# anton-galkovsky/pointcloudTraj

Measured on AMD Instinct MI355X. Metric: nn_queries_per_sec_10M_point_cloud, higher is better.
Workload: dtype f64; 1 GPU; C3-throughput: 10000000 uniform fp32 points in [0,100.0)^3 (seed 3), 1048576 uniform NN queries per step (4 distinct batches in rotation, seeds [5, 1005, 2005, 3005]), grid kernel, inputs resident in HBM; points_per_gpu=10000000, total_points=10000000, algo=grid, query_batches_in_rotation=4, gpu_work_before_the_warmup_steps=none, full=False, parallelism=single GPU, cards=1

## Files before the change

pointcloudtraj_amd/build.py:

```python
from __future__ import annotations

import os
import shutil
import subprocess

PKG = os.path.dirname(os.path.abspath(__file__))
ROOT = os.path.dirname(PKG)
CSRC = os.path.join(PKG, "csrc")
LIB = os.path.join(PKG, "lib")
ENGINE_SO = os.environ.get("PCT_ENGINE_SO") or os.path.join(LIB, "libpct_engine.so")
KDTREE_SO = os.path.join(LIB, "libkdtree.so")
DEMO_BIN = os.path.join(LIB, "seam_demo")
NODE_BIN = os.path.join(LIB, "node_call_sites")
CORRIDOR_SO = os.path.join(LIB, "libpct_corridor.so")
SHARD_SO = os.path.join(LIB, "libpct_shard.so")
SHARD_CLIENT = os.path.join(LIB, "shard_client")

HIPCC = shutil.which("hipcc") or "/opt/rocm/bin/hipcc"
COMMON = ["-O3", "--offload-arch=gfx950", "-std=c++17", "-fPIC", "-shared", "-ffp-contract=off",
          "-Wall", "-Wno-unused-function", "-I" + os.path.join(ROOT, "include")]


def _stale(target: str, sources: list[str]) -> bool:
    if not os.path.exists(target):
        return True
    t = os.path.getmtime(target)
    return any(os.path.getmtime(s) > t for s in sources)


def build_all(force: bool = False, verbose: bool = False) -> None:
    os.makedirs(LIB, exist_ok=True)
    hdrs = [os.path.join(ROOT, "include", "pct_engine.h"), os.path.join(ROOT, "include", "kdtree", "kdtree.h"),
            os.path.join(ROOT, "include", "kdtree", "kdtree_ext.h")]
    hdrs += [os.path.join(ROOT, "include", "pct_voxel.h"), os.path.join(ROOT, "include", "pct_traj.h")]
    eng_units = [os.path.join(CSRC, "engine.hip"), os.path.join(CSRC, "voxel.hip"), os.path.join(CSRC, "traj.hip"), os.path.join(CSRC, "nodeset.hip")]
    eng_src = eng_units + [os.path.join(CSRC, f) for f in ("kernels.hpp", "gridbuild.hpp", "pyramid.hpp", "bernstein.hpp", "brute2.hpp", "knn.hpp", "rsearch.hpp", "ring.hpp", "ring_dedup.hpp", "vox_key.hpp", "ring_search.hpp", "ring_host.inc", "engine_internal.hpp")]
    if force or _stale(ENGINE_SO, eng_src + hdrs):
        cmd = [HIPCC, *COMMON, "-o", ENGINE_SO, *eng_units]
        if verbose:
            print(" ".join(cmd))
        subprocess.run(cmd, check=True)
    kd_src = [os.path.join(CSRC, "kdtree_gpu.cpp")]
    if os.path.exists(kd_src[0]) and (force or _stale(KDTREE_SO, kd_src + hdrs + [ENGINE_SO])):
        cmd = ["g++", "-O2", "-std=c++17", "-fPIC", "-shared", "-Wall", "-ffp-contract=off", "-I" + os.path.join(ROOT, "include"),
               "-o", KDTREE_SO, kd_src[0], "-L" + LIB, "-lpct_engine", "-Wl,-rpath,$ORIGIN", "-Wl,-soname,libkdtree.so"]
        if verbose:
            print(" ".join(cmd))
        subprocess.run(cmd, check=True)


    cor_src = os.path.join(CSRC, "corridor.cpp")
    cor_hdrs = [os.path.join(ROOT, "include", h) for h in ("pct_corridor.h", "pct_corridor_finder.hpp", "pct_obstacle_map.hpp")]
    if os.path.exists(cor_src) and os.path.exists(KDTREE_SO) and (force or _stale(CORRIDOR_SO, [cor_src, KDTREE_SO] + cor_hdrs + hdrs)):
        cmd = ["g++", "-O2", "-std=c++17", "-fPIC", "-shared", "-Wall", "-ffp-contract=off", "-I" + os.path.join(ROOT, "include"),
               "-o", CORRIDOR_SO, cor_src, "-L" + LIB, "-lkdtree", "-lpct_engine", "-Wl,-rpath,$ORIGIN", "-Wl,-rpath-link," + LIB,
               "-L/opt/rocm/lib", "-Wl,-rpath-link,/opt/rocm/lib", "-Wl,-soname,libpct_corridor.so"]
        if verbose:
            print(" ".join(cmd))
        subprocess.run(cmd, check=True)
# ... 57 lines not shown
```

pointcloudtraj_amd/csrc/engine.hip:

```cpp
#include <hip/hip_runtime.h>
#include <hip/hip_ext.h>

#include <algorithm>
#include <chrono>
#include <cmath>
#include <cstdarg>
#include <cstdio>
#include <cstdlib>
#include <cstring>
#include <type_traits>
#include <vector>

#include "../../include/pct_engine.h"
#include "engine_internal.hpp"
#include "kernels.hpp"
#include "gridbuild.hpp"
#include "pyramid.hpp"
#include "ring.hpp"
#include "ring_dedup.hpp"
#include "brute2.hpp"
#include "knn.hpp"
#include "rsearch.hpp"
#include "ring_search.hpp"

// ... 126 lines not shown
    ExpandOut *h_eout = nullptr, *d_eout = nullptr;
    double *h_bpos = nullptr, *d_bpos = nullptr;
    unsigned char *d_stage = nullptr;
    size_t stage_bytes = 0;
    float *d_bbox = nullptr;
    GbCheck *d_gbcheck = nullptr, *h_gbcheck = nullptr;
    GbCheck last_check{};
    bool has_pyr = false;
    PyrDesc P{};
    PyrNode *pyr_nodes = nullptr;
    unsigned char *pyr_hint = nullptr;
    size_t pyr_cap = 0, pyr_total = 0, pyr_hint_cap = 0;
    double empty_frac = 0.0;
    bool was_sparse = false;
    bool has_grid = false;
    GridDesc G{};
    uint32_t *cell_start = nullptr;
    size_t cells_cap = 0;
    float4 *sorted = nullptr;
    size_t sorted_cap = 0;
    uint4 *blocks = nullptr;
    size_t blocks_cap = 0;
    BinDesc B{};
    float4 *d_qsorted = nullptr;
    uint32_t *d_sort1 = nullptr;
    int sort_phase = 0;
    int64_t qcap = 0;
    float *d_q = nullptr, *d_r = nullptr;
    double *d_q64 = nullptr, *d_r2 = nullptr, *d_d2 = nullptr, *d_radius = nullptr, *d_pts64 = nullptr;
    uint32_t *d_idx = nullptr, *d_count = nullptr, *d_bound = nullptr;
    uint32_t *d_todo = nullptr;
    unsigned char *d_skip = nullptr;
    double *d_part_d2 = nullptr;
    uint32_t *d_part_idx = nullptr;
    int64_t part_q = 0;
    uint32_t *d_ovf = nullptr;
    uint32_t *d_cand_count = nullptr, *d_cand_idx = nullptr;
    double *d_cand_d2 = nullptr;
    uint32_t *d_knn_idx = nullptr, *d_knn_pidx = nullptr;
    double *d_knn_d2 = nullptr, *d_knn_pd2 = nullptr;
    size_t knn_out_cap = 0, knn_part_cap = 0;
    long long *rs_off = nullptr;
    uint64_t *rs_tiles = nullptr;
    uint32_t *rs_cursor = nullptr, *rs_queue = nullptr;
    int64_t rs_qcap = 0;
    uint32_t *rs_idx = nullptr;
// ... 519 lines not shown
    const double *d_q64 = c->d_q64 + 3 * qoff;
    d_idx += qoff;
    d_d2 += qoff;
    const int blocks = stream_blocks(c->count, Q);
    return launch_frame(c, s, Q, { Work::EveryPoint }, no_step,
        [&] {
            for_each_query_tile(Q, [&](auto qt, int q0, int qcount) {
                nn_stream_kernel<decltype(qt)::value><<<blocks, 256, 0, s>>>(c->x, c->y, c->z, (uint32_t)c->count, d_q64, q0, qcount, c->d_part_d2,
                                                                             c->d_part_idx, blocks);
            });
        },
        [&] {
            nn_reduce_partials_kernel<<<(int)Q, 256, 0, s>>>(c->d_part_d2, c->d_part_idx, blocks, (uint32_t)c->index_base, d_idx, d_d2);
        });
}

int nn_stream_q64(pct_cloud *c, int64_t Q, uint32_t *d_idx, double *d_d2, hipStream_t s)
{
    for (int64_t off = 0; off < Q; off += c->part_q) PCTCHK(nn_stream_q64_slice(c, off, std::min<int64_t>(c->part_q, Q - off), d_idx, d_d2, s));
    c->host_points = (uint64_t)Q * (uint64_t)c->count;
    return PCT_OK;
}

int bin_queries(pct_cloud *c, const float *d_q, int64_t Q, hipStream_t s, const float4 **recs_out)
{
    *recs_out = nullptr;
    if (Q < 16384) return PCT_OK;
    const BinDesc &B = c->B;
    int key_shift = 0;
    while ((((uint64_t)B.nbins - 1) >> key_shift) >= (1ull << 20)) key_shift++;
    const bool pingpong = !c->capturing;
    uint32_t *total1 = c->d_sort1 + (c->sort_phase ? kSortBuckets : 0), *total1_next = c->d_sort1 + (c->sort_phase ? 0 : kSortBuckets);
    uint32_t *fill1 = c->d_sort1 + 2 * kSortBuckets;
    const uint32_t per_block = (uint32_t)std::min<int64_t>(kSortPerBlock, std::max<int64_t>(1024, (Q / 128 + 1023) / 1024 * 1024));
    const int nb = ceil_div(Q, (int64_t)per_block);
    with_bool((reinterpret_cast<uintptr_t>(d_q) & 15u) == 0, [&](auto aligned) {
        constexpr bool A = decltype(aligned)::value;
        qsort_hist_kernel<A><<<nb, 1024, 0, s>>>(c->G, B, key_shift, d_q, (uint32_t)Q, per_block, total1, fill1, pingpong ? total1_next : nullptr);
        qsort_scatter1_kernel<A><<<nb, 1024, 0, s>>>(c->G, B, key_shift, d_q, (uint32_t)Q, per_block, total1, fill1, c->d_qsorted);
    });
    if (pingpong) c->sort_phase ^= 1;
    else HIPCHK(hipMemsetAsync(total1, 0, sizeof(uint32_t) * kSortBuckets, s));
    HIPCHK(hipGetLastError());
    *recs_out = c->d_qsorted;
    return PCT_OK;
}

int g_filter_mode = -1;

int cloud_bbox_cached(pct_cloud *c)
{
    if (c->bbox_epoch == c->content_epoch) return PCT_OK;
    hipStream_t s = g_stream;
    const int64_t n = c->count;
    const int bblocks = (int)std::min<int64_t>(1024, (n + 255) / 256);
    float *d_part = c->d_bbox;
    bbox_partial_kernel<<<bblocks, 256, 0, s>>>(c->x, c->y, c->z, (uint32_t)n, d_part);
    std::vector<float> part((size_t)bblocks * 6);
    hipError_t e = hipMemcpyAsync(part.data(), d_part, part.size() * sizeof(float), hipMemcpyDeviceToHost, s);
    if (e == hipSuccess) e = hipStreamSynchronize(s);
    if (e != hipSuccess) return fail(PCT_ERR_HIP, "bbox reduction failed: %s", hipGetErrorString(e));
    for (int k = 0; k < 3; k++) { c->bbox_lo[k] = INFINITY; c->bbox_hi[k] = -INFINITY; }
// ... 147 lines not shown
        return fail(PCT_ERR_INVALID, "unknown algo %d", algo);
    }
    if (op == Op::KNN && *path == Path::Stream && c->capturing)
        return fail(PCT_ERR_INVALID, "the streaming k-NN kernel is not available during graph capture");
    if (c->count == 0) *path = Path::Empty;
    return PCT_OK;
}

int nn_run(pct_cloud *c, Path path, const float *d_q, int64_t Q, uint32_t *d_idx, double *d_d2, hipStream_t s)
{
    switch (path) {
    case Path::Empty:
        fill_empty_kernel<<<ceil_div(Q, 256), 256, 0, s>>>(d_idx, d_d2, (uint32_t)Q);
        HIPCHK(hipGetLastError());
        return PCT_OK;
    case Path::Table:
        return launch_frame(c, s, Q, { Work::DeviceKept }, [&] {
            ring_batch_kernel<false><<<(int)Q, 256, 0, s>>>(ring_view(c), InflateParams{}, d_q, nullptr, (double)INFINITY, (uint32_t)c->index_base, d_idx, d_d2,
                                                            nullptr, nullptr, ExpressSignal{});
        });
    case Path::Grid: {
        const float4 *recs = nullptr;
        const int blocks = ceil_div(Q, 256 / kCoop);
        return launch_frame(c, s, Q, { Work::Device, Dom::Ext }, [&] { return bin_queries(c, d_q, Q, s, &recs); },
            [&] {
                with_bool(c->count_work, [&](auto count_work) {
                    constexpr bool CW = decltype(count_work)::value;
                    if (c->has_pyr) {
                        launch_dominant(c, s, nn_grid_pyr_kernel<CW>, blocks, c->G, c->P, c->pyr_nodes, c->pyr_hint, c->sorted, c->cell_start, d_q, (uint32_t)Q,
                                        (uint32_t)c->index_base, recs, d_idx, d_d2, c->d_work, c->d_todo);
                        nn_grid_pyr_todo_kernel<CW><<<(int)std::min<int64_t>(256, blocks), 256, 0, s>>>(c->G, c->P, c->pyr_nodes, c->pyr_hint, c->sorted, c->cell_start, d_q,
                                                                                                        (uint32_t)c->index_base, recs, d_idx, d_d2, c->d_work, c->d_todo);
                    } else
                        launch_dominant(c, s, nn_grid_coop_kernel<CW>, blocks, c->G, c->sorted, c->cell_start, d_q, (uint32_t)Q, (uint32_t)c->index_base, recs, d_idx,
                                        d_d2, c->d_work);
                });
            }, no_step);
    }
    default:
        widen_queries_kernel<<<ceil_div(3 * Q, 256), 256, 0, s>>>(d_q, (uint32_t)(3 * Q), c->d_q64);
        if (path == Path::StreamExact) return nn_stream_q64(c, Q, d_idx, d_d2, s);
        return nn_stream_filtered(c, d_q, Q, d_idx, d_d2, s);
    }
}

int nn_dev(pct_cloud *c, int algo, const float *d_q, int64_t Q, uint32_t *d_idx, double *d_d2, hipStream_t s)
{
    if (Q == 0) return PCT_OK;
    if (Q > c->qcap) return fail(PCT_ERR_INVALID, "batch of %lld exceeds reserved %lld (call pct_cloud_reserve_queries)", (long long)Q, (long long)c->qcap);
    Path path;
    PCTCHK(resolve_algo(c, Op::NN, algo, Q, &path));
    return nn_run(c, path, d_q, Q, d_idx, d_d2, s);
}

int count_run(pct_cloud *c, Path path, const float *d_q, const float *d_r, int64_t Q, uint32_t *d_count, hipStream_t s)
{
    HIPCHK(hipMemsetAsync(d_count, 0, sizeof(uint32_t) * Q, s));
    switch (path) {
// ... 372 lines not shown
        if (c->hx) (void)hipHostFree(c->hx);
        if (c->hy) (void)hipHostFree(c->hy);
        if (c->hz) (void)hipHostFree(c->hz);
        c->x = c->y = c->z = nullptr;
    }
    if (c->h_xout) (void)hipHostFree(c->h_xout);
    if (c->h_xin) (void)hipHostFree(c->h_xin);
    if (c->h_xr) (void)hipHostFree(c->h_xr);
    if (c->h_xids) (void)hipHostFree(c->h_xids);
    if (c->h_xseq) (void)hipHostFree(c->h_xseq);
    if (c->ev_mut) (void)hipEventDestroy(c->ev_mut);
    if (c->h_frame) (void)hipHostFree(c->h_frame);
    if (c->h_astage) (void)hipHostFree(c->h_astage);
    if (c->h_mq) (void)hipHostFree(c->h_mq);
    if (c->h_mi) (void)hipHostFree(c->h_mi);
    if (c->h_md) (void)hipHostFree(c->h_md);
    dev_free(c->d_xcounter);
    if (c->h_aux) (void)hipHostFree(c->h_aux);
    if (c->h_eout) (void)hipHostFree(c->h_eout);
    if (c->h_bpos) (void)hipHostFree(c->h_bpos);
    dev_free(c->x); dev_free(c->y); dev_free(c->z); dev_free(c->d_stage); dev_free(c->gb_tmp); dev_free(c->gb_small);
    dev_free(c->blocks);
    dev_free(c->cell_start); dev_free(c->sorted);
    dev_free(c->d_qsorted); dev_free(c->d_sort1); dev_free(c->d_todo);
    dev_free(c->d_q); dev_free(c->d_r); dev_free(c->d_q64); dev_free(c->d_r2); dev_free(c->d_d2); dev_free(c->d_radius);
    dev_free(c->d_pts64); dev_free(c->d_idx); dev_free(c->d_count); dev_free(c->d_skip); dev_free(c->d_bound);
    dev_free(c->d_part_d2); dev_free(c->d_part_idx); dev_free(c->d_cand_count); dev_free(c->d_cand_d2); dev_free(c->d_cand_idx); dev_free(c->d_ovf);
    dev_free(c->d_coef); dev_free(c->d_segtime); dev_free(c->d_orders); dev_free(c->d_nsamples); dev_free(c->d_first_hit);
    dev_free(c->d_work);
    dev_free(c->d_knn_idx); dev_free(c->d_knn_d2); dev_free(c->d_knn_pidx); dev_free(c->d_knn_pd2);
    dev_free(c->rs_off); dev_free(c->rs_tiles); dev_free(c->rs_cursor); dev_free(c->rs_queue); dev_free(c->rs_idx); dev_free(c->rs_d2);
    dev_free(c->d_bbox); dev_free(c->d_gbcheck); dev_free(c->pyr_nodes); dev_free(c->pyr_hint);
    if (c->h_gbcheck) (void)hipHostFree(c->h_gbcheck);
    dev_free(c->ring_ht); dev_free(c->ring_slots); dev_free(c->ring_ovf); dev_free(c->ring_where); dev_free(c->ring_st);
    if (c->h_ring_status) (void)hipHostFree(c->h_ring_status);
    dev_free(c->dd_keys); dev_free(c->dd_vals); dev_free(c->dd_pslot); dev_free(c->dd_rank); dev_free(c->dd_tile); dev_free(c->dd_flags); dev_free(c->dd_out);
    if (c->h_dd_word) (void)hipHostFree(c->h_dd_word);
    replan_ctx_free(c->rp);
    dev_free(c->crop_tile); dev_free(c->crop_idx); dev_free(c->crop_d2); dev_free(c->crop_x); dev_free(c->crop_y); dev_free(c->crop_z);
    if (c->ev0) (void)hipEventDestroy(c->ev0);
    if (c->ev1) (void)hipEventDestroy(c->ev1);
    for (hipEvent_t e : c->dom_ring) if (e) (void)hipEventDestroy(e);
    delete c;
    return PCT_OK;
}

int64_t pct_cloud_size(const pct_cloud *c) { return c ? c->count : 0; }
// ... 73 lines not shown

extern "C" {

int pct_cloud_append_aos(pct_cloud *c, const void *pts, int64_t n, int64_t stride_bytes)
{
    if (!c || n < 0 || (n > 0 && !pts) || stride_bytes < 12 || (stride_bytes & 3)) return fail(PCT_ERR_INVALID, "bad append arguments");
    if (n > c->cap) return fail(PCT_ERR_CAPACITY, "appending %lld points to a ring of %lld", (long long)n, (long long)c->cap);
    if (c->ring_on && c->dd_res > 0) return ring_append_dedup(c, pts, n, stride_bytes);
    if (n == 0) return PCT_OK;
    drop_grid(c);
    if (c->ring_ready) return ring_append(c, pts, n, stride_bytes);
    return append_unindexed(c, pts, n, stride_bytes);
}

int pct_cloud_reserve_queries(pct_cloud *c, int64_t Q)
{
    if (!c || Q < 0) return fail(PCT_ERR_INVALID, "bad reserve");
    if (Q <= c->qcap) return PCT_OK;
    if (c->capturing) return fail(PCT_ERR_INVALID, "cannot grow workspaces during graph capture");
    HIPCHK(hipStreamSynchronize(g_stream));
    const int64_t q = std::max<int64_t>(Q, 256);
    dev_free(c->d_q); dev_free(c->d_r); dev_free(c->d_q64); dev_free(c->d_r2); dev_free(c->d_d2); dev_free(c->d_radius);
    dev_free(c->d_pts64); dev_free(c->d_idx); dev_free(c->d_count); dev_free(c->d_skip); dev_free(c->d_bound);
    dev_free(c->d_part_d2); dev_free(c->d_part_idx); dev_free(c->d_cand_count); dev_free(c->d_cand_d2); dev_free(c->d_cand_idx); dev_free(c->d_ovf); dev_free(c->d_qsorted); dev_free(c->d_todo);
    c->qcap = 0;
    c->generation++;
    PCTCHK(dev_alloc(&c->d_q, 3 * q));
    PCTCHK(dev_alloc(&c->d_r, q));
    PCTCHK(dev_alloc(&c->d_q64, 3 * q));
    PCTCHK(dev_alloc(&c->d_r2, q));
    PCTCHK(dev_alloc(&c->d_d2, q));
    PCTCHK(dev_alloc(&c->d_radius, q));
    PCTCHK(dev_alloc(&c->d_pts64, 3 * q));
    PCTCHK(dev_alloc(&c->d_idx, q));
    PCTCHK(dev_alloc(&c->d_count, q));
    PCTCHK(dev_alloc(&c->d_skip, q));
    PCTCHK(dev_alloc(&c->d_bound, q));
    PCTCHK(dev_alloc(&c->d_qsorted, q));
    PCTCHK(dev_alloc(&c->d_todo, 2 * q + 16));
    HIPCHK(hipMemset(c->d_todo, 0, sizeof(uint32_t) * 16));
    if (!c->d_sort1) {
        PCTCHK(dev_alloc(&c->d_sort1, 3 * kSortBuckets));
        HIPCHK(hipMemset(c->d_sort1, 0, sizeof(uint32_t) * 3 * kSortBuckets));
    }
    c->part_q = std::min<int64_t>(q, kPartQueries);
    PCTCHK(dev_alloc(&c->d_part_d2, (size_t)c->part_q * kMaxParts));
    PCTCHK(dev_alloc(&c->d_part_idx, (size_t)c->part_q * kMaxParts));
    PCTCHK(dev_alloc(&c->d_ovf, (size_t)c->part_q + 1));
    PCTCHK(dev_alloc(&c->d_cand_count, (size_t)c->part_q));
    PCTCHK(dev_alloc(&c->d_cand_d2, (size_t)c->part_q * kCandCap));
    PCTCHK(dev_alloc(&c->d_cand_idx, (size_t)c->part_q * kCandCap));
    HIPCHK(hipMemset(c->d_cand_count, 0, sizeof(uint32_t) * (size_t)c->part_q));
    c->qcap = q;
    return PCT_OK;
}

int pct_cloud_drop_grid(pct_cloud *c)
{
    if (!c) return fail(PCT_ERR_INVALID, "null cloud");
    drop_grid(c);
    return PCT_OK;
// ... 1076 lines not shown
```

pointcloudtraj_amd/csrc/kernels.hpp:

```cpp
#pragma once
#include <hip/hip_runtime.h>
#include <stdint.h>

#pragma clang fp contract(off)

#include "bernstein.hpp"

namespace pct {

constexpr int kWave = 64;
constexpr uint32_t kNoIndex = 0xFFFFFFFFu;

__device__ __forceinline__ double dist2(double px, double py, double pz, double qx, double qy, double qz)
{
    double dx = px - qx, dy = py - qy, dz = pz - qz;
    double s = dx * dx;
    s = s + dy * dy;
    s = s + dz * dz;
    return s;
}

__device__ __forceinline__ bool better(double d2a, uint32_t ia, double d2b, uint32_t ib)
{
    return d2a < d2b || (d2a == d2b && ia < ib);
}

__device__ __forceinline__ uint32_t reported_index(double d2, uint32_t i, uint32_t index_base)
{
    return (i == kNoIndex || !(d2 < __builtin_huge_val())) ? kNoIndex : i + index_base;
// ... 684 lines not shown
}

__global__ __launch_bounds__(256) void square_radii_kernel(const float *__restrict__ r, uint32_t n, double *__restrict__ r2)
{
    const uint32_t i = blockIdx.x * blockDim.x + threadIdx.x;
    if (i < n) { const double w = (double)r[i]; r2[i] = w * w; }
}

__global__ __launch_bounds__(256) void fill_empty_kernel(uint32_t *__restrict__ idx, double *__restrict__ d2, uint32_t n)
{
    const uint32_t i = blockIdx.x * blockDim.x + threadIdx.x;
    if (i < n) { idx[i] = kNoIndex; d2[i] = __builtin_huge_val(); }
}

struct GridDesc {
    float ox, oy, oz, inv_h;
    double oxd, oyd, ozd, hd;
    int gx, gy, gz;
    uint32_t ncells;
    int octant_first;
    const uint4 *blocks;
};

__device__ __forceinline__ int cell_coord(float v, float o, float inv_h, int g)
{
    float t = floorf((v - o) * inv_h);
    t = fminf(fmaxf(t, 0.0f), (float)(g - 1));
    return (int)t;
}

__device__ __forceinline__ uint32_t cell_lin(const GridDesc &G, int cx, int cy, int cz)
{
    return ((uint32_t)cz * (uint32_t)G.gy + (uint32_t)cy) * (uint32_t)G.gx + (uint32_t)cx;
}

__global__ __launch_bounds__(256) void block_corner_kernel(GridDesc G, const uint32_t *__restrict__ cell_start, uint4 *__restrict__ blocks, uint32_t ncorners)
{
    const uint32_t i = blockIdx.x * blockDim.x + threadIdx.x;
    if (i >= ncorners) return;
    const uint32_t ux = (uint32_t)G.gx + 1u, uy = (uint32_t)G.gy + 1u;
    const int u = (int)(i % ux), v = (int)((i / ux) % uy), w = (int)(i / (ux * uy));
    const int xa = max(u - 1, 0), xb = min(u, G.gx - 1), ya = max(v - 1, 0), yb = min(v, G.gy - 1), za = max(w - 1, 0), zb = min(w, G.gz - 1);
    uint32_t s[4], e[4];
#pragma unroll
    for (int r = 0; r < 4; r++) {
        const bool ok = !((r >> 1) && zb == za) && !((r & 1) && yb == ya);
        const uint32_t row = cell_lin(G, 0, (r & 1) ? yb : ya, (r >> 1) ? zb : za);
        s[r] = cell_start[row + xa];
        e[r] = ok ? cell_start[row + xb + 1] : s[r];
    }
    blocks[2u * i] = make_uint4(s[0], s[1], s[2], s[3]);
    blocks[2u * i + 1u] = make_uint4(e[0], e[1], e[2], e[3]);
// ... 196 lines not shown
    if (blockIdx.x == 0)
        for (int i = threadIdx.x; i < kSortBuckets; i += 1024) {
            fill1[i] = 0;
            if (total1_next) total1_next[i] = 0;
        }
    for (int i = threadIdx.x; i < kSortBuckets; i += 1024) h[i] = 0;
    __syncthreads();
    const uint32_t base = blockIdx.x * per_block;
    const int items = (int)(per_block >> 10);
    float qv[kSortItems][3];
    sort_load_items<VEC>(q, base, threadIdx.x, items, Q, qv);
#pragma unroll
    for (int k = 0; k < kSortItems; k++) {
        if (sort_item_live<VEC>(base, k, threadIdx.x, items, Q)) {
            const uint32_t key = query_bin(G, B, qv[k][0], qv[k][1], qv[k][2]) >> key_shift;
            atomicAdd(&h[key >> kSortLShift], 1u);
        }
    }
    __syncthreads();
    for (int i = threadIdx.x; i < kSortBuckets; i += 1024)
        if (h[i]) atomicAdd(&total1[i], h[i]);
}

template <bool VEC>
__global__ __launch_bounds__(1024) void qsort_scatter1_kernel(GridDesc G, BinDesc B, int key_shift, const float *__restrict__ q,
                                                              uint32_t Q, uint32_t per_block, const uint32_t *__restrict__ total1,
                                                              uint32_t *__restrict__ fill1, float4 *__restrict__ qsorted)
{
    static_assert(kSortBuckets == 1024, "one thread per bucket");
    __shared__ uint32_t h[kSortBuckets];
    __shared__ uint32_t basepos[kSortBuckets];
    __shared__ uint32_t s_wave[16];
    h[threadIdx.x] = 0;
    const uint32_t tot = total1[threadIdx.x];
    const int lane = threadIdx.x & 63, wave = threadIdx.x >> 6;
    uint32_t inc = tot;
#pragma unroll
    for (int off = 1; off < 64; off <<= 1) {
        const uint32_t o = (uint32_t)__shfl_up((int)inc, off, kWave);
        if (lane >= off) inc += o;
    }
    if (lane == 63) s_wave[wave] = inc;
    __syncthreads();
    uint32_t start = inc - tot;
    for (int w = 0; w < wave; w++) start += s_wave[w];
    const uint32_t base = blockIdx.x * per_block;
    const int items = (int)(per_block >> 10);
    uint32_t key[kSortItems];
    float qv[kSortItems][3];
    sort_load_items<VEC>(q, base, threadIdx.x, items, Q, qv);
#pragma unroll
    for (int k = 0; k < kSortItems; k++)
        key[k] = sort_item_live<VEC>(base, k, threadIdx.x, items, Q) ? query_bin(G, B, qv[k][0], qv[k][1], qv[k][2]) >> key_shift : 0xFFFFFFFFu;
    uint32_t rank[kSortItems];
#pragma unroll
    for (int k = 0; k < kSortItems; k++)
        if (key[k] != 0xFFFFFFFFu) rank[k] = atomicAdd(&h[key[k] >> kSortLShift], 1u);
    __syncthreads();
    {
        const uint32_t mine = h[threadIdx.x];
        basepos[threadIdx.x] = mine ? start + atomicAdd(&fill1[threadIdx.x], mine) : 0u;
    }
    __syncthreads();
#pragma unroll
    for (int k = 0; k < kSortItems; k++) {
        if (key[k] != 0xFFFFFFFFu) {
            const uint32_t t = sort_item<VEC>(base, k, threadIdx.x);
            const uint32_t pos = basepos[key[k] >> kSortLShift] + rank[k];
            qsorted[pos] = make_float4(qv[k][0], qv[k][1], qv[k][2], __uint_as_float(t));
        }
    }
}

struct WorkCounters { unsigned long long points, cells, nodes; };
constexpr int kWorkSlots = 64;

__device__ __forceinline__ uint32_t xcd_contiguous_block(uint32_t b, uint32_t nblocks)
{
    const uint32_t xcd = b & 7u, k = b >> 3;
    const uint32_t q = nblocks >> 3, r = nblocks & 7u;
    return (xcd < r ? xcd * (q + 1) : r * (q + 1) + (xcd - r) * q) + k;
}

__device__ __forceinline__ double cube_bound(const GridDesc &G, int cx, int cy, int cz, int r, double qx, double qy, double qz)
{
    double bound = __builtin_huge_val();
    if (cx - r > 0) bound = fmin(bound, qx - (G.oxd + (double)(cx - r) * G.hd));
    if (cx + r < G.gx - 1) bound = fmin(bound, (G.oxd + (double)(cx + r + 1) * G.hd) - qx);
    if (cy - r > 0) bound = fmin(bound, qy - (G.oyd + (double)(cy - r) * G.hd));
    if (cy + r < G.gy - 1) bound = fmin(bound, (G.oyd + (double)(cy + r + 1) * G.hd) - qy);
    if (cz - r > 0) bound = fmin(bound, qz - (G.ozd + (double)(cz - r) * G.hd));
    if (cz + r < G.gz - 1) bound = fmin(bound, (G.ozd + (double)(cz + r + 1) * G.hd) - qz);
// ... 54 lines not shown
        const bool zface = (zz == cz - r) || (zz == cz + r);
        for (int yy = y0; yy <= y1; yy++) {
            const uint32_t row = cell_lin(G, 0, yy, zz);
            if (full || zface || yy == cy - r || yy == cy + r) {
                const uint32_t s = cell_start[row + x0], e = cell_start[row + x1 + 1];
                if (COUNT && sub == 0) { npts += e - s; nruns += 1; }
                coop_scan_exact(pts, s, e, sub, qx, qy, qz, bd, bi);
            } else {
                if (cx - r >= 0) {
                    const uint32_t s = cell_start[row + cx - r], e = cell_start[row + cx - r + 1];
                    if (COUNT && sub == 0) { npts += e - s; nruns += 1; }
                    coop_scan_exact(pts, s, e, sub, qx, qy, qz, bd, bi);
                }
                if (cx + r <= G.gx - 1) {
                    const uint32_t s = cell_start[row + cx + r], e = cell_start[row + cx + r + 1];
                    if (COUNT && sub == 0) { npts += e - s; nruns += 1; }
                    coop_scan_exact(pts, s, e, sub, qx, qy, qz, bd, bi);
                }
            }
        }
    }
}

template <int NR, int DEPTH>
__device__ __forceinline__ void coop_screen_rows(const float4 *__restrict__ pts, const uint32_t (&rs)[NR], const uint32_t (&re)[NR],
                                                 uint32_t sub, float qxf, float qyf, float qzf, double qx, double qy, double qz,
                                                 double &bd, uint32_t &bi)
{
    float m1 = __builtin_huge_valf(), m2 = __builtin_huge_valf();
    uint32_t p1 = 0;
    float4 P[NR][DEPTH];
#pragma unroll
    for (int k = 0; k < NR; k++) {
        const uint32_t a = rs[k], b = re[k];
        const uint32_t last = b > a ? b - 1 : 0u;
#pragma unroll
        for (int j = 0; j < DEPTH; j++) P[k][j] = pts[min(a + sub + kCoop * j, last)];
    }
#pragma unroll
    for (int k = 0; k < NR; k++) {
        const uint32_t a = rs[k], b = re[k];
#pragma unroll
        for (int j = 0; j < DEPTH; j++) {
            const uint32_t p = a + sub + kCoop * j;
            const float dx = P[k][j].x - qxf, dy = P[k][j].y - qyf, dz = P[k][j].z - qzf;
            float d = __builtin_fmaf(dz, dz, __builtin_fmaf(dy, dy, dx * dx));
            d = (p < b) ? d : __builtin_huge_valf();
            const bool lt = d < m1;
            m2 = __builtin_amdgcn_fmed3f(m1, m2, d);
            p1 = lt ? p : p1;
            m1 = fminf(m1, d);
        }
    }
    auto long_row = [&](uint32_t a, uint32_t b) {
        for (uint32_t p = a + kCoop * DEPTH + sub; p < b; p += kCoop) {
            const float4 Pp = pts[p];
            const float dx = Pp.x - qxf, dy = Pp.y - qyf, dz = Pp.z - qzf;
            const float d = __builtin_fmaf(dz, dz, __builtin_fmaf(dy, dy, dx * dx));
            const bool lt = d < m1;
            m2 = __builtin_amdgcn_fmed3f(m1, m2, d);
            p1 = lt ? p : p1;
// ... 89 lines not shown
            }
            if (COUNT) {
                npts += my_e - my_s; nruns += ok ? 1u : 0u;
            }
        }
        uint32_t rs[9], re[9];
#pragma unroll
        for (int k = 0; k < 8; k++) { rs[k] = (uint32_t)__shfl((int)my_s, k, kCoop); re[k] = (uint32_t)__shfl((int)my_e, k, kCoop); }
        rs[8] = s8; re[8] = e8;

        coop_screen_rows<9, 1>(pts, rs, re, sub, qxf, qyf, qzf, qx, qy, qz, bd, bi);
    }
    for (int r = 1;; r++) {
        if (r > 1) {
            coop_scan_cube_or_shell<COUNT>(G, pts, cell_start, cx, cy, cz, r, false, sub, qx, qy, qz, bd, bi, npts, nruns);
            coop_argmin8(bd, bi);
        }
        const double bound = cube_bound(G, cx, cy, cz, r, qx, qy, qz);
        if (bound == __builtin_huge_val() || (bound > 0.0 && bd <= bound * bound)) break;
    }
}


__device__ __forceinline__ bool block_leaves_undecided(const GridDesc &G, int cx, int cy, int cz, int xa, int xb, int ya, int yb, int za, int zb,
                                                       float fx, float fy, float fz, double qx, double qy, double qz, double bd)
{
    {
        const float inf = __builtin_huge_valf();
        float bc = inf;
        bc = fminf(bc, xa > 0 ? fx + (float)(cx - xa) : inf);
        bc = fminf(bc, xb < G.gx - 1 ? (float)(xb + 1 - cx) - fx : inf);
        bc = fminf(bc, ya > 0 ? fy + (float)(cy - ya) : inf);
        bc = fminf(bc, yb < G.gy - 1 ? (float)(yb + 1 - cy) - fy : inf);
        bc = fminf(bc, za > 0 ? fz + (float)(cz - za) : inf);
        bc = fminf(bc, zb < G.gz - 1 ? (float)(zb + 1 - cz) - fz : inf);
        if (bc < inf && fmaxf(fmaxf(fabsf(fx), fabsf(fy)), fabsf(fz)) < 2.0f) {
            const double b = (double)((bc - 0.015625f) * (float)G.hd * 0.999999f);
            if (b > 0.0 && bd <= b * b) return false;
        }
    }
    double bound = __builtin_huge_val();
    if (xa > 0) bound = fmin(bound, qx - (G.oxd + (double)xa * G.hd));
    if (xb < G.gx - 1) bound = fmin(bound, (G.oxd + (double)(xb + 1) * G.hd) - qx);
    if (ya > 0) bound = fmin(bound, qy - (G.oyd + (double)ya * G.hd));
    if (yb < G.gy - 1) bound = fmin(bound, (G.oyd + (double)(yb + 1) * G.hd) - qy);
    if (za > 0) bound = fmin(bound, qz - (G.ozd + (double)za * G.hd));
    if (zb < G.gz - 1) bound = fmin(bound, (G.ozd + (double)(zb + 1) * G.hd) - qz);
    if (bound == __builtin_huge_val()) return false;
    bound -= G.hd * (1.0 / 256.0);
    return !(bound > 0.0 && bd <= bound * bound);
}

template <bool COUNT>
__device__ __forceinline__ bool coop_stage0(const GridDesc &G, const float4 *__restrict__ pts, const uint32_t *__restrict__ cell_start,
                                            float qxf, float qyf, float qzf, uint32_t sub, double &bd, uint32_t &bi, uint32_t &npts,
                                            uint32_t &nruns)
{
    const double qx = (double)qxf, qy = (double)qyf, qz = (double)qzf;
    const int cx = cell_coord(qxf, G.ox, G.inv_h, G.gx);
    const int cy = cell_coord(qyf, G.oy, G.inv_h, G.gy);
    const int cz = cell_coord(qzf, G.oz, G.inv_h, G.gz);
    const float fx = (qxf - G.ox) * G.inv_h - (float)cx, fy = (qyf - G.oy) * G.inv_h - (float)cy, fz = (qzf - G.oz) * G.inv_h - (float)cz;
    const int xa = max(fx < 0.5f ? cx - 1 : cx, 0), xb = min(fx < 0.5f ? cx : cx + 1, G.gx - 1);
    const int ya = max(fy < 0.5f ? cy - 1 : cy, 0), yb = min(fy < 0.5f ? cy : cy + 1, G.gy - 1);
    const int za = max(fz < 0.5f ? cz - 1 : cz, 0), zb = min(fz < 0.5f ? cz : cz + 1, G.gz - 1);
    uint32_t rs[4], re[4];
    if (G.blocks) {
        const uint32_t u = (uint32_t)(fx < 0.5f ? cx : cx + 1), v = (uint32_t)(fy < 0.5f ? cy : cy + 1), w = (uint32_t)(fz < 0.5f ? cz : cz + 1);
        const uint4 *ent = G.blocks + 2u * ((w * ((uint32_t)G.gy + 1u) + v) * ((uint32_t)G.gx + 1u) + u);
        const uint4 S = ent[0], E = ent[1];
        rs[0] = S.x; rs[1] = S.y; rs[2] = S.z; rs[3] = S.w;
        re[0] = E.x; re[1] = E.y; re[2] = E.z; re[3] = E.w;
        if (COUNT && sub < 4) {
            const int ri = (int)sub;
            const bool ok = !((ri >> 1) && zb == za) && !((ri & 1) && yb == ya);
            npts += re[ri] - rs[ri]; nruns += ok ? 1u : 0u;
        }
    } else {
        const int ri = (int)sub & 3;
        const bool ok = !((ri >> 1) && zb == za) && !((ri & 1) && yb == ya);
        const uint32_t row = cell_lin(G, 0, (ri & 1) ? yb : ya, (ri >> 1) ? zb : za);
        const uint32_t a = cell_start[row + xa], b = cell_start[row + xb + 1];
        const uint32_t my_s = a, my_e = ok ? b : a;
        if (COUNT && sub < 4) { npts += my_e - my_s; nruns += ok ? 1u : 0u; }
#pragma unroll
        for (int k = 0; k < 4; k++) { rs[k] = (uint32_t)__shfl((int)my_s, k, kCoop); re[k] = (uint32_t)__shfl((int)my_e, k, kCoop); }
    }
    coop_screen_rows<4, 2>(pts, rs, re, sub, qxf, qyf, qzf, qx, qy, qz, bd, bi);
    return block_leaves_undecided(G, cx, cy, cz, xa, xb, ya, yb, za, zb, fx, fy, fz, qx, qy, qz, bd);
}

template <bool COUNT>
__device__ __forceinline__ void wave_cube_search(const GridDesc &G, const float4 *__restrict__ pts, const uint32_t *__restrict__ cell_start,
                                                 float qxf, float qyf, float qzf, double &bd, uint32_t &bi, uint32_t &npts, uint32_t &nruns)
{
    const uint32_t lane = threadIdx.x & 63;
    const double qx = (double)qxf, qy = (double)qyf, qz = (double)qzf;
    const int cx = cell_coord(qxf, G.ox, G.inv_h, G.gx);
    const int cy = cell_coord(qyf, G.oy, G.inv_h, G.gy);
    const int cz = cell_coord(qzf, G.oz, G.inv_h, G.gz);
    const int x0 = max(cx - 1, 0), x1 = min(cx + 1, G.gx - 1);
    uint32_t my_s, my_e;
    {
        const int l = lane < 9 ? (int)lane : 0;
        const int zz = cz + l / 3 - 1, yy = cy + l % 3 - 1;
        const bool ok = zz >= 0 && zz < G.gz && yy >= 0 && yy < G.gy;
        const uint32_t row = ok ? cell_lin(G, 0, yy, zz) : 0u;
        const uint32_t a = cell_start[row + x0], b = cell_start[row + x1 + 1];
        my_s = a;
        my_e = ok ? b : a;
        if (COUNT && lane < 9) { npts += my_e - my_s; nruns += ok ? 1u : 0u; }
    }
// ... 60 lines not shown
        wave_argmin(bd, bi);
    }
}

template <bool COUNT>
__device__ __forceinline__ void coop_finish_shells(const GridDesc &G, const float4 *__restrict__ pts, const uint32_t *__restrict__ cell_start,
                                                   float qxf, float qyf, float qzf, uint32_t sub, double &bd, uint32_t &bi, uint32_t &npts,
                                                   uint32_t &nruns)
{
    const double qx = (double)qxf, qy = (double)qyf, qz = (double)qzf;
    const int cx = cell_coord(qxf, G.ox, G.inv_h, G.gx);
    const int cy = cell_coord(qyf, G.oy, G.inv_h, G.gy);
    const int cz = cell_coord(qzf, G.oz, G.inv_h, G.gz);
    for (int r = 1;; r++) {
        if (r > 1) {
            coop_scan_cube_or_shell<COUNT>(G, pts, cell_start, cx, cy, cz, r, false, sub, qx, qy, qz, bd, bi, npts, nruns);
            coop_argmin8(bd, bi);
        }
        const double bound = cube_bound(G, cx, cy, cz, r, qx, qy, qz);
        if (bound == __builtin_huge_val() || (bound > 0.0 && bd <= bound * bound)) break;
    }
}

template <bool COUNT>
__device__ __forceinline__ void coop_wave_search(const GridDesc &G, const float4 *__restrict__ pts, const uint32_t *__restrict__ cell_start, bool live,
                                                 float qxf, float qyf, float qzf, uint32_t sub, double &bd, uint32_t &bi, uint32_t &npts, uint32_t &nruns)
{
    bd = __builtin_huge_val();
    bi = kNoIndex;
    bool undecided = false;
    if (live) undecided = coop_stage0<COUNT>(G, pts, cell_start, qxf, qyf, qzf, sub, bd, bi, npts, nruns);
    unsigned long long todo = __builtin_amdgcn_ballot_w64(undecided && sub == 0);
    while (todo) {
        const int g = __builtin_ctzll(todo);
        todo &= todo - 1;
        const float bx = __uint_as_float((uint32_t)__builtin_amdgcn_readlane((int)__float_as_uint(qxf), g)),
                    by = __uint_as_float((uint32_t)__builtin_amdgcn_readlane((int)__float_as_uint(qyf), g)),
                    bz = __uint_as_float((uint32_t)__builtin_amdgcn_readlane((int)__float_as_uint(qzf), g));
        double cbd;
        uint32_t cbi;
        wave_cube_search<COUNT>(G, pts, cell_start, bx, by, bz, cbd, cbi, npts, nruns);
        if (((threadIdx.x & 63) >> 3) == (uint32_t)(g >> 3)) { bd = cbd; bi = cbi; }
    }
    if (live && undecided) coop_finish_shells<COUNT>(G, pts, cell_start, qxf, qyf, qzf, sub, bd, bi, npts, nruns);
}

template <bool COUNT>
__global__ __launch_bounds__(256) __attribute__((amdgpu_waves_per_eu(7, 7))) void nn_grid_coop_kernel(GridDesc G, const float4 *__restrict__ pts,
                                                           const uint32_t *__restrict__ cell_start,
                                                           const float *__restrict__ q, uint32_t Q, uint32_t index_base,
                                                           const float4 *__restrict__ qsorted,
                                                           uint32_t *__restrict__ out_idx, double *__restrict__ out_d2,
                                                           WorkCounters *__restrict__ work)
{
    const uint32_t sub = threadIdx.x & (kCoop - 1);
    const uint32_t bslot = qsorted ? xcd_contiguous_block(blockIdx.x, gridDim.x) : blockIdx.x;
    const uint32_t slot = bslot * (256 / kCoop) + (threadIdx.x / kCoop);
    uint32_t npts = 0, nruns = 0;
    if (G.octant_first) {
        const bool live = slot < Q;
        uint32_t t = slot;
        float qxf = 0.0f, qyf = 0.0f, qzf = 0.0f;
        if (live) {
            if (qsorted) {
                const float4 R = qsorted[slot];
                qxf = R.x; qyf = R.y; qzf = R.z; t = __float_as_uint(R.w);
            } else {
                qxf = q[3 * t]; qyf = q[3 * t + 1]; qzf = q[3 * t + 2];
            }
        }
        double bd;
        uint32_t bi;
        coop_wave_search<COUNT>(G, pts, cell_start, live, qxf, qyf, qzf, sub, bd, bi, npts, nruns);
        if (live && sub == 0) {
            out_idx[t] = reported_index(bd, bi, index_base);
            out_d2[t] = bd;
        }
    } else if (slot < Q) {
        uint32_t t = slot;
        float qxf, qyf, qzf;
        if (qsorted) {
            const float4 R = qsorted[slot];
            qxf = R.x; qyf = R.y; qzf = R.z; t = __float_as_uint(R.w);
        } else {
            qxf = q[3 * t]; qyf = q[3 * t + 1]; qzf = q[3 * t + 2];
        }
        double bd;
        uint32_t bi;
        coop_nn_search<COUNT>(G, pts, cell_start, qxf, qyf, qzf, sub, bd, bi, npts, nruns);
        if (sub == 0) {
            out_idx[t] = reported_index(bd, bi, index_base);
            out_d2[t] = bd;
        }
    }
    if (COUNT) {
        unsigned long long a = npts, b = nruns;
// ... 517 lines not shown
```

Baseline: 7.729 billion queries/s.

## Precompute per-query stage0 descriptors during binning scatter for grid NN search

The query-sort scatter kernel now also writes a 16-byte descriptor per sorted query, holding the base cell row, the y/z row steps, the span and the early-accept threshold. The coop NN kernel loads this descriptor instead of recomputing cell coordinates and block bounds before issuing its cell_start loads, shortening the dependent chain ahead of the first memory access. An empty asm fence forces all eight point loads to issue before the screening math. The cost is an extra 16 B write and read per query, and a full block recomputation when the fast threshold test fails.

```diff
diff --git a/pointcloudtraj_amd/build.py b/pointcloudtraj_amd/build.py
--- a/pointcloudtraj_amd/build.py
+++ b/pointcloudtraj_amd/build.py
@@ -34,7 +34,7 @@
             os.path.join(ROOT, "include", "kdtree", "kdtree_ext.h")]
     hdrs += [os.path.join(ROOT, "include", "pct_voxel.h"), os.path.join(ROOT, "include", "pct_traj.h")]
     eng_units = [os.path.join(CSRC, "engine.hip"), os.path.join(CSRC, "voxel.hip"), os.path.join(CSRC, "traj.hip"), os.path.join(CSRC, "nodeset.hip")]
-    eng_src = eng_units + [os.path.join(CSRC, f) for f in ("kernels.hpp", "gridbuild.hpp", "pyramid.hpp", "bernstein.hpp", "brute2.hpp", "knn.hpp", "rsearch.hpp", "ring.hpp", "ring_dedup.hpp", "vox_key.hpp", "ring_search.hpp", "ring_host.inc", "engine_internal.hpp")]
+    eng_src = eng_units + [os.path.join(CSRC, f) for f in ("kernels.hpp", "gridbuild.hpp", "pyramid.hpp", "bernstein.hpp", "brute2.hpp", "knn.hpp", "rsearch.hpp", "ring.hpp", "ring_dedup.hpp", "vox_key.hpp", "ring_search.hpp", "ring_host.inc", "engine_internal.hpp", "stage0_desc.hpp")]
     if force or _stale(ENGINE_SO, eng_src + hdrs):
         cmd = [HIPCC, *COMMON, "-o", ENGINE_SO, *eng_units]
         if verbose:
diff --git a/pointcloudtraj_amd/csrc/engine.hip b/pointcloudtraj_amd/csrc/engine.hip
--- a/pointcloudtraj_amd/csrc/engine.hip
+++ b/pointcloudtraj_amd/csrc/engine.hip
@@ -172,6 +172,7 @@
     uint4 *blocks = nullptr;
     size_t blocks_cap = 0;
     BinDesc B{};
+    Stage0Desc *d_qgeom = nullptr;
     float4 *d_qsorted = nullptr;
     uint32_t *d_sort1 = nullptr;
     int sort_phase = 0;
@@ -737,7 +738,7 @@
     return PCT_OK;
 }
 
-int bin_queries(pct_cloud *c, const float *d_q, int64_t Q, hipStream_t s, const float4 **recs_out)
+int bin_queries(pct_cloud *c, const float *d_q, int64_t Q, hipStream_t s, const float4 **recs_out, bool want_desc = false)
 {
     *recs_out = nullptr;
     if (Q < 16384) return PCT_OK;
@@ -752,7 +753,8 @@
     with_bool((reinterpret_cast<uintptr_t>(d_q) & 15u) == 0, [&](auto aligned) {
         constexpr bool A = decltype(aligned)::value;
         qsort_hist_kernel<A><<<nb, 1024, 0, s>>>(c->G, B, key_shift, d_q, (uint32_t)Q, per_block, total1, fill1, pingpong ? total1_next : nullptr);
-        qsort_scatter1_kernel<A><<<nb, 1024, 0, s>>>(c->G, B, key_shift, d_q, (uint32_t)Q, per_block, total1, fill1, c->d_qsorted);
+        if (want_desc) qsort_scatter1_kernel<A, true><<<nb, 1024, 0, s>>>(c->G, B, key_shift, d_q, (uint32_t)Q, per_block, total1, fill1, c->d_qsorted, c->d_qgeom);
+        else qsort_scatter1_kernel<A, false><<<nb, 1024, 0, s>>>(c->G, B, key_shift, d_q, (uint32_t)Q, per_block, total1, fill1, c->d_qsorted, nullptr);
     });
     if (pingpong) c->sort_phase ^= 1;
     else HIPCHK(hipMemsetAsync(total1, 0, sizeof(uint32_t) * kSortBuckets, s));
@@ -946,7 +948,8 @@
     case Path::Grid: {
         const float4 *recs = nullptr;
         const int blocks = ceil_div(Q, 256 / kCoop);
-        return launch_frame(c, s, Q, { Work::Device, Dom::Ext }, [&] { return bin_queries(c, d_q, Q, s, &recs); },
+        const bool want_desc = !c->has_pyr && c->G.octant_first && c->G.blocks == nullptr && std::max(c->G.gx, c->G.gy) <= kStage0MaxAxis;
+        return launch_frame(c, s, Q, { Work::Device, Dom::Ext }, [&] { return bin_queries(c, d_q, Q, s, &recs, want_desc); },
             [&] {
                 with_bool(c->count_work, [&](auto count_work) {
                     constexpr bool CW = decltype(count_work)::value;
@@ -956,8 +959,11 @@
                         nn_grid_pyr_todo_kernel<CW><<<(int)std::min<int64_t>(256, blocks), 256, 0, s>>>(c->G, c->P, c->pyr_nodes, c->pyr_hint, c->sorted, c->cell_start, d_q,
                                                                                                         (uint32_t)c->index_base, recs, d_idx, d_d2, c->d_work, c->d_todo);
                     } else
-                        launch_dominant(c, s, nn_grid_coop_kernel<CW>, blocks, c->G, c->sorted, c->cell_start, d_q, (uint32_t)Q, (uint32_t)c->index_base, recs, d_idx,
-                                        d_d2, c->d_work);
+                        with_bool(recs && want_desc, [&](auto desc) {
+                            constexpr bool DS = decltype(desc)::value;
+                            launch_dominant(c, s, nn_grid_coop_kernel<CW, DS>, blocks, c->G, c->sorted, c->cell_start, d_q, (uint32_t)Q, (uint32_t)c->index_base, recs,
+                                            DS ? c->d_qgeom : nullptr, d_idx, d_d2, c->d_work);
+                        });
                 });
             }, no_step);
     }
@@ -1376,7 +1382,7 @@
     dev_free(c->x); dev_free(c->y); dev_free(c->z); dev_free(c->d_stage); dev_free(c->gb_tmp); dev_free(c->gb_small);
     dev_free(c->blocks);
     dev_free(c->cell_start); dev_free(c->sorted);
-    dev_free(c->d_qsorted); dev_free(c->d_sort1); dev_free(c->d_todo);
+    dev_free(c->d_qsorted); dev_free(c->d_qgeom); dev_free(c->d_sort1); dev_free(c->d_todo);
     dev_free(c->d_q); dev_free(c->d_r); dev_free(c->d_q64); dev_free(c->d_r2); dev_free(c->d_d2); dev_free(c->d_radius);
     dev_free(c->d_pts64); dev_free(c->d_idx); dev_free(c->d_count); dev_free(c->d_skip); dev_free(c->d_bound);
     dev_free(c->d_part_d2); dev_free(c->d_part_idx); dev_free(c->d_cand_count); dev_free(c->d_cand_d2); dev_free(c->d_cand_idx); dev_free(c->d_ovf);
@@ -1496,7 +1502,7 @@
     const int64_t q = std::max<int64_t>(Q, 256);
     dev_free(c->d_q); dev_free(c->d_r); dev_free(c->d_q64); dev_free(c->d_r2); dev_free(c->d_d2); dev_free(c->d_radius);
     dev_free(c->d_pts64); dev_free(c->d_idx); dev_free(c->d_count); dev_free(c->d_skip); dev_free(c->d_bound);
-    dev_free(c->d_part_d2); dev_free(c->d_part_idx); dev_free(c->d_cand_count); dev_free(c->d_cand_d2); dev_free(c->d_cand_idx); dev_free(c->d_ovf); dev_free(c->d_qsorted); dev_free(c->d_todo);
+    dev_free(c->d_part_d2); dev_free(c->d_part_idx); dev_free(c->d_cand_count); dev_free(c->d_cand_d2); dev_free(c->d_cand_idx); dev_free(c->d_ovf); dev_free(c->d_qsorted); dev_free(c->d_qgeom); dev_free(c->d_todo);
     c->qcap = 0;
     c->generation++;
     PCTCHK(dev_alloc(&c->d_q, 3 * q));
@@ -1511,6 +1517,7 @@
     PCTCHK(dev_alloc(&c->d_skip, q));
     PCTCHK(dev_alloc(&c->d_bound, q));
     PCTCHK(dev_alloc(&c->d_qsorted, q));
+    PCTCHK(dev_alloc(&c->d_qgeom, q));
     PCTCHK(dev_alloc(&c->d_todo, 2 * q + 16));
     HIPCHK(hipMemset(c->d_todo, 0, sizeof(uint32_t) * 16));
     if (!c->d_sort1) {
diff --git a/pointcloudtraj_amd/csrc/kernels.hpp b/pointcloudtraj_amd/csrc/kernels.hpp
--- a/pointcloudtraj_amd/csrc/kernels.hpp
+++ b/pointcloudtraj_amd/csrc/kernels.hpp
@@ -5,6 +5,7 @@
 #pragma clang fp contract(off)
 
 #include "bernstein.hpp"
+#include "stage0_desc.hpp"
 
 namespace pct {
 
@@ -735,12 +736,6 @@
     const uint4 *blocks;
 };
 
-__device__ __forceinline__ int cell_coord(float v, float o, float inv_h, int g)
-{
-    float t = floorf((v - o) * inv_h);
-    t = fminf(fmaxf(t, 0.0f), (float)(g - 1));
-    return (int)t;
-}
 
 __device__ __forceinline__ uint32_t cell_lin(const GridDesc &G, int cx, int cy, int cz)
 {
@@ -983,10 +978,11 @@
         if (h[i]) atomicAdd(&total1[i], h[i]);
 }
 
-template <bool VEC>
+template <bool VEC, bool DESC>
 __global__ __launch_bounds__(1024) void qsort_scatter1_kernel(GridDesc G, BinDesc B, int key_shift, const float *__restrict__ q,
                                                               uint32_t Q, uint32_t per_block, const uint32_t *__restrict__ total1,
-                                                              uint32_t *__restrict__ fill1, float4 *__restrict__ qsorted)
+                                                              uint32_t *__restrict__ fill1, float4 *__restrict__ qsorted,
+                                                              Stage0Desc *__restrict__ qdesc)
 {
     static_assert(kSortBuckets == 1024, "one thread per bucket");
     __shared__ uint32_t h[kSortBuckets];
@@ -1029,6 +1025,7 @@
             const uint32_t t = sort_item<VEC>(base, k, threadIdx.x);
             const uint32_t pos = basepos[key[k] >> kSortLShift] + rank[k];
             qsorted[pos] = make_float4(qv[k][0], qv[k][1], qv[k][2], __uint_as_float(t));
+            if (DESC) qdesc[pos] = stage0_desc(G, qv[k][0], qv[k][1], qv[k][2]);
         }
     }
 }
@@ -1129,7 +1126,7 @@
     }
 }
 
-template <int NR, int DEPTH>
+template <int NR, int DEPTH, bool FENCE = false>
 __device__ __forceinline__ void coop_screen_rows(const float4 *__restrict__ pts, const uint32_t (&rs)[NR], const uint32_t (&re)[NR],
                                                  uint32_t sub, float qxf, float qyf, float qzf, double qx, double qy, double qz,
                                                  double &bd, uint32_t &bi)
@@ -1144,6 +1141,15 @@
 #pragma unroll
         for (int j = 0; j < DEPTH; j++) P[k][j] = pts[min(a + sub + kCoop * j, last)];
     }
+#if defined(__HIP_DEVICE_COMPILE__)
+    if constexpr (FENCE) {
+        static_assert(NR * DEPTH == 8, "the operand list below is written out for eight points");
+        asm volatile("" :: "v"(P[0][0].x), "v"(P[0][0].y), "v"(P[0][0].z), "v"(P[0][1].x), "v"(P[0][1].y), "v"(P[0][1].z),
+                           "v"(P[1][0].x), "v"(P[1][0].y), "v"(P[1][0].z), "v"(P[1][1].x), "v"(P[1][1].y), "v"(P[1][1].z),
+                           "v"(P[2][0].x), "v"(P[2][0].y), "v"(P[2][0].z), "v"(P[2][1].x), "v"(P[2][1].y), "v"(P[2][1].z),
+                           "v"(P[3][0].x), "v"(P[3][0].y), "v"(P[3][0].z), "v"(P[3][1].x), "v"(P[3][1].y), "v"(P[3][1].z));
+    }
+#endif
 #pragma unroll
     for (int k = 0; k < NR; k++) {
         const uint32_t a = rs[k], b = re[k];
@@ -1279,23 +1285,9 @@
 }
 
 
-__device__ __forceinline__ bool block_leaves_undecided(const GridDesc &G, int cx, int cy, int cz, int xa, int xb, int ya, int yb, int za, int zb,
-                                                       float fx, float fy, float fz, double qx, double qy, double qz, double bd)
-{
-    {
-        const float inf = __builtin_huge_valf();
-        float bc = inf;
-        bc = fminf(bc, xa > 0 ? fx + (float)(cx - xa) : inf);
-        bc = fminf(bc, xb < G.gx - 1 ? (float)(xb + 1 - cx) - fx : inf);
-        bc = fminf(bc, ya > 0 ? fy + (float)(cy - ya) : inf);
-        bc = fminf(bc, yb < G.gy - 1 ? (float)(yb + 1 - cy) - fy : inf);
-        bc = fminf(bc, za > 0 ? fz + (float)(cz - za) : inf);
-        bc = fminf(bc, zb < G.gz - 1 ? (float)(zb + 1 - cz) - fz : inf);
-        if (bc < inf && fmaxf(fmaxf(fabsf(fx), fabsf(fy)), fabsf(fz)) < 2.0f) {
-            const double b = (double)((bc - 0.015625f) * (float)G.hd * 0.999999f);
-            if (b > 0.0 && bd <= b * b) return false;
-        }
-    }
+__device__ __forceinline__ bool block_bound_undecided(const GridDesc &G, int xa, int xb, int ya, int yb, int za, int zb, double qx, double qy,
+                                                      double qz, double bd)
+{
     double bound = __builtin_huge_val();
     if (xa > 0) bound = fmin(bound, qx - (G.oxd + (double)xa * G.hd));
     if (xb < G.gx - 1) bound = fmin(bound, (G.oxd + (double)(xb + 1) * G.hd) - qx);
@@ -1308,19 +1300,22 @@
     return !(bound > 0.0 && bd <= bound * bound);
 }
 
+__device__ __forceinline__ bool block_leaves_undecided(const GridDesc &G, const Stage0Block &K, double qx, double qy, double qz, double bd)
+{
+    const double b = (double)stage0_accept_threshold(G, K);
+    if (b > 0.0 && bd <= b * b) return false;
+    return block_bound_undecided(G, K.xa, K.xb, K.ya, K.yb, K.za, K.zb, qx, qy, qz, bd);
+}
+
 template <bool COUNT>
 __device__ __forceinline__ bool coop_stage0(const GridDesc &G, const float4 *__restrict__ pts, const uint32_t *__restrict__ cell_start,
                                             float qxf, float qyf, float qzf, uint32_t sub, double &bd, uint32_t &bi, uint32_t &npts,
                                             uint32_t &nruns)
 {
     const double qx = (double)qxf, qy = (double)qyf, qz = (double)qzf;
-    const int cx = cell_coord(qxf, G.ox, G.inv_h, G.gx);
-    const int cy = cell_coord(qyf, G.oy, G.inv_h, G.gy);
-    const int cz = cell_coord(qzf, G.oz, G.inv_h, G.gz);
-    const float fx = (qxf - G.ox) * G.inv_h - (float)cx, fy = (qyf - G.oy) * G.inv_h - (float)cy, fz = (qzf - G.oz) * G.inv_h - (float)cz;
-    const int xa = max(fx < 0.5f ? cx - 1 : cx, 0), xb = min(fx < 0.5f ? cx : cx + 1, G.gx - 1);
-    const int ya = max(fy < 0.5f ? cy - 1 : cy, 0), yb = min(fy < 0.5f ? cy : cy + 1, G.gy - 1);
-    const int za = max(fz < 0.5f ? cz - 1 : cz, 0), zb = min(fz < 0.5f ? cz : cz + 1, G.gz - 1);
+    const Stage0Block K = stage0_block(G, qxf, qyf, qzf);
+    const int cx = K.cx, cy = K.cy, cz = K.cz, xa = K.xa, xb = K.xb, ya = K.ya, yb = K.yb, za = K.za, zb = K.zb;
+    const float fx = K.fx, fy = K.fy, fz = K.fz;
     uint32_t rs[4], re[4];
     if (G.blocks) {
         const uint32_t u = (uint32_t)(fx < 0.5f ? cx : cx + 1), v = (uint32_t)(fy < 0.5f ? cy : cy + 1), w = (uint32_t)(fz < 0.5f ? cz : cz + 1);
@@ -1344,7 +1339,31 @@
         for (int k = 0; k < 4; k++) { rs[k] = (uint32_t)__shfl((int)my_s, k, kCoop); re[k] = (uint32_t)__shfl((int)my_e, k, kCoop); }
     }
     coop_screen_rows<4, 2>(pts, rs, re, sub, qxf, qyf, qzf, qx, qy, qz, bd, bi);
-    return block_leaves_undecided(G, cx, cy, cz, xa, xb, ya, yb, za, zb, fx, fy, fz, qx, qy, qz, bd);
+    return block_leaves_undecided(G, K, qx, qy, qz, bd);
+}
+
+template <bool COUNT>
+__device__ __forceinline__ bool coop_stage0_desc(const GridDesc &G, const float4 *__restrict__ pts, const uint32_t *__restrict__ cell_start,
+                                                 const Stage0Desc &D, float qxf, float qyf, float qzf, uint32_t sub, double &bd, uint32_t &bi,
+                                                 uint32_t &npts, uint32_t &nruns)
+{
+    const double qx = (double)qxf, qy = (double)qyf, qz = (double)qzf;
+    uint32_t rs[4], re[4];
+    {
+        const int ri = (int)sub & 3;
+        const uint32_t ystep = D.ystep_span & 0xFFFFu, span = D.ystep_span >> 16, zstep = D.zstep;
+        const bool ok = !((ri >> 1) && zstep == 0u) && !((ri & 1) && ystep == 0u);
+        const uint32_t row = D.cell + ((ri & 1) ? ystep : 0u) + ((ri >> 1) ? zstep : 0u);
+        const uint32_t a = cell_start[row], b = cell_start[row + span];
+        const uint32_t my_s = a, my_e = ok ? b : a;
+        if (COUNT && sub < 4) { npts += my_e - my_s; nruns += ok ? 1u : 0u; }
+#pragma unroll
+        for (int k = 0; k < 4; k++) { rs[k] = (uint32_t)__shfl((int)my_s, k, kCoop); re[k] = (uint32_t)__shfl((int)my_e, k, kCoop); }
+    }
+    coop_screen_rows<4, 2, true>(pts, rs, re, sub, qxf, qyf, qzf, qx, qy, qz, bd, bi);
+    if (D.thr > 0.0f && bd <= (double)D.thr * (double)D.thr) return false;
+    const Stage0Block K = stage0_block(G, qxf, qyf, qzf);
+    return block_bound_undecided(G, K.xa, K.xb, K.ya, K.yb, K.za, K.zb, qx, qy, qz, bd);
 }
 
 template <bool COUNT>
@@ -1451,14 +1470,18 @@
     }
 }
 
-template <bool COUNT>
+template <bool COUNT, bool DESC>
 __device__ __forceinline__ void coop_wave_search(const GridDesc &G, const float4 *__restrict__ pts, const uint32_t *__restrict__ cell_start, bool live,
-                                                 float qxf, float qyf, float qzf, uint32_t sub, double &bd, uint32_t &bi, uint32_t &npts, uint32_t &nruns)
+                                                 const Stage0Desc &D, float qxf, float qyf, float qzf, uint32_t sub, double &bd,
+                                                 uint32_t &bi, uint32_t &npts, uint32_t &nruns)
 {
     bd = __builtin_huge_val();
     bi = kNoIndex;
     bool undecided = false;
-    if (live) undecided = coop_stage0<COUNT>(G, pts, cell_start, qxf, qyf, qzf, sub, bd, bi, npts, nruns);
+    if (live) {
+        if (DESC) undecided = coop_stage0_desc<COUNT>(G, pts, cell_start, D, qxf, qyf, qzf, sub, bd, bi, npts, nruns);
+        else undecided = coop_stage0<COUNT>(G, pts, cell_start, qxf, qyf, qzf, sub, bd, bi, npts, nruns);
+    }
     unsigned long long todo = __builtin_amdgcn_ballot_w64(undecided && sub == 0);
     while (todo) {
         const int g = __builtin_ctzll(todo);
@@ -1474,11 +1497,11 @@
     if (live && undecided) coop_finish_shells<COUNT>(G, pts, cell_start, qxf, qyf, qzf, sub, bd, bi, npts, nruns);
 }
 
-template <bool COUNT>
+template <bool COUNT, bool DESC>
 __global__ __launch_bounds__(256) __attribute__((amdgpu_waves_per_eu(7, 7))) void nn_grid_coop_kernel(GridDesc G, const float4 *__restrict__ pts,
                                                            const uint32_t *__restrict__ cell_start,
                                                            const float *__restrict__ q, uint32_t Q, uint32_t index_base,
-                                                           const float4 *__restrict__ qsorted,
+                                                           const float4 *__restrict__ qsorted, const Stage0Desc *__restrict__ qdesc,
                                                            uint32_t *__restrict__ out_idx, double *__restrict__ out_d2,
                                                            WorkCounters *__restrict__ work)
 {
@@ -1490,9 +1513,11 @@
         const bool live = slot < Q;
         uint32_t t = slot;
         float qxf = 0.0f, qyf = 0.0f, qzf = 0.0f;
+        Stage0Desc D{};
         if (live) {
             if (qsorted) {
                 const float4 R = qsorted[slot];
+                if (DESC) D = qdesc[slot];
                 qxf = R.x; qyf = R.y; qzf = R.z; t = __float_as_uint(R.w);
             } else {
                 qxf = q[3 * t]; qyf = q[3 * t + 1]; qzf = q[3 * t + 2];
@@ -1500,7 +1525,7 @@
         }
         double bd;
         uint32_t bi;
-        coop_wave_search<COUNT>(G, pts, cell_start, live, qxf, qyf, qzf, sub, bd, bi, npts, nruns);
+        coop_wave_search<COUNT, DESC>(G, pts, cell_start, live, D, qxf, qyf, qzf, sub, bd, bi, npts, nruns);
         if (live && sub == 0) {
             out_idx[t] = reported_index(bd, bi, index_base);
             out_d2[t] = bd;
diff --git a/pointcloudtraj_amd/csrc/stage0_desc.hpp b/pointcloudtraj_amd/csrc/stage0_desc.hpp
--- /dev/null
+++ b/pointcloudtraj_amd/csrc/stage0_desc.hpp
@@ -0,0 +1,73 @@
+#pragma once
+#include <cmath>
+#include <cstdint>
+
+#if defined(__HIPCC__)
+#define PCT_HD __host__ __device__
+#else
+#define PCT_HD
+#endif
+
+PCT_HD inline int cell_coord(float v, float o, float inv_h, int g)
+{
+    float t = floorf((v - o) * inv_h);
+    t = fminf(fmaxf(t, 0.0f), (float)(g - 1));
+    return (int)t;
+}
+
+struct alignas(16) Stage0Desc {
+    uint32_t cell;
+    uint32_t ystep_span;
+    uint32_t zstep;
+    float thr;
+};
+static_assert(sizeof(Stage0Desc) == 16, "one 16-byte load per query");
+
+constexpr int kStage0MaxAxis = 1024;
+static_assert(kStage0MaxAxis < (1 << 16) && (int64_t)kStage0MaxAxis * kStage0MaxAxis < (1ll << 32), "row steps of the descriptor");
+
+PCT_HD inline int s0_max(int a, int b) { return a > b ? a : b; }
+PCT_HD inline int s0_min(int a, int b) { return a < b ? a : b; }
+
+struct Stage0Block { int cx, cy, cz, xa, xb, ya, yb, za, zb; float fx, fy, fz; };
+
+template <class Grid>
+PCT_HD inline Stage0Block stage0_block(const Grid &G, float qxf, float qyf, float qzf)
+{
+    Stage0Block K;
+    K.cx = cell_coord(qxf, G.ox, G.inv_h, G.gx);
+    K.cy = cell_coord(qyf, G.oy, G.inv_h, G.gy);
+    K.cz = cell_coord(qzf, G.oz, G.inv_h, G.gz);
+    K.fx = (qxf - G.ox) * G.inv_h - (float)K.cx; K.fy = (qyf - G.oy) * G.inv_h - (float)K.cy; K.fz = (qzf - G.oz) * G.inv_h - (float)K.cz;
+    K.xa = s0_max(K.fx < 0.5f ? K.cx - 1 : K.cx, 0); K.xb = s0_min(K.fx < 0.5f ? K.cx : K.cx + 1, G.gx - 1);
+    K.ya = s0_max(K.fy < 0.5f ? K.cy - 1 : K.cy, 0); K.yb = s0_min(K.fy < 0.5f ? K.cy : K.cy + 1, G.gy - 1);
+    K.za = s0_max(K.fz < 0.5f ? K.cz - 1 : K.cz, 0); K.zb = s0_min(K.fz < 0.5f ? K.cz : K.cz + 1, G.gz - 1);
+    return K;
+}
+
+template <class Grid>
+PCT_HD inline float stage0_accept_threshold(const Grid &G, const Stage0Block &K)
+{
+    const float inf = __builtin_huge_valf();
+    float bc = inf;
+    bc = fminf(bc, K.xa > 0 ? K.fx + (float)(K.cx - K.xa) : inf);
+    bc = fminf(bc, K.xb < G.gx - 1 ? (float)(K.xb + 1 - K.cx) - K.fx : inf);
+    bc = fminf(bc, K.ya > 0 ? K.fy + (float)(K.cy - K.ya) : inf);
+    bc = fminf(bc, K.yb < G.gy - 1 ? (float)(K.yb + 1 - K.cy) - K.fy : inf);
+    bc = fminf(bc, K.za > 0 ? K.fz + (float)(K.cz - K.za) : inf);
+    bc = fminf(bc, K.zb < G.gz - 1 ? (float)(K.zb + 1 - K.cz) - K.fz : inf);
+    if (bc < inf && fmaxf(fmaxf(fabsf(K.fx), fabsf(K.fy)), fabsf(K.fz)) < 2.0f) return (bc - 0.015625f) * (float)G.hd * 0.999999f;
+    return 0.0f;
+}
+
+template <class Grid>
+PCT_HD inline Stage0Desc stage0_desc(const Grid &G, float qxf, float qyf, float qzf)
+{
+    const Stage0Block K = stage0_block(G, qxf, qyf, qzf);
+    Stage0Desc D;
+    D.cell = ((uint32_t)K.za * (uint32_t)G.gy + (uint32_t)K.ya) * (uint32_t)G.gx + (uint32_t)K.xa;
+    D.ystep_span = (K.yb > K.ya ? (uint32_t)G.gx : 0u) | ((uint32_t)(K.xb - K.xa + 1) << 16);
+    D.zstep = K.zb > K.za ? (uint32_t)G.gx * (uint32_t)G.gy : 0u;
+    D.thr = stage0_accept_threshold(G, K);
+    return D;
+}
```

New measurement: 7.409 billion queries/s. 4.1% lower.
